# adelowo/cap

Hardware: AMD Instinct MI355X
Metric: verified JWTs/sec (RS256-2048, ES256) at 1/2/4/8 MI355X vs all-core Go CPU (higher is better)
Workload: dtype u32 (28-bit limbs, 64-bit v_mad_u64_u32 accumulators); 1 GPU; ES256 P-256 JWKS with 4 kids, 1M tokens batch-verified per MI355X (BASELINE configs[1]); kids=4, p256_key_comb_w=26, parallelism=independent shards x1

## Files before the change

### cap_amd/csrc/kernels/ec_small.hpp

```cpp
#pragma once
#include "ecdsa_impl.hpp"
#include "small_common.hpp"

namespace {

constexpr int SM_SPLIT = 16;
constexpr uint32_t SM_SIG_CHARS = 176;

__device__ __forceinline__ int sm_hash_bits(int alg) { return alg == 7 ? 256 : alg == 8 ? 384 : 512; }

template <class CV>
__device__ __forceinline__ void jadd_pair(JPt<typename CV::Fp>& P, int off, bool& exc) {
  using Fp = typename CV::Fp;
  constexpr int L = Fp::L;
  const bool lo = (threadIdx.x & off) == 0;
  uint32_t oz[L], ox[L], oy[L];
#pragma unroll
  for (int j = 0; j < L; ++j) {
    ox[j] = __shfl_xor(P.X[j], off);
    oy[j] = __shfl_xor(P.Y[j], off);
    oz[j] = __shfl_xor(P.Z[j], off);
  }
  const bool oinf = __shfl_xor((int)P.inf, off) != 0;
  const int pexc = __shfl_xor((int)exc, off);
// ... 126 lines not shown
  const bool size_ok = nch <= SM_SIG_CHARS && (nch & 3u) != 1u && D == 2u * (uint32_t)ks;
  if (wave == 1 && size_ok) {
    if (sm_b64_decode(sig_w, sig_shift, nch, sig_b, lane) && lane == 0) flag[0] = 1;
  }
  __syncthreads();

  if (wave == 1 && size_ok) {
    const int q = lane & 31, half = lane >> 5;
    if (q < CW) {
      uint32_t w = 0;
#pragma unroll
      for (int b = 0; b < 4; ++b) {
        const int pos = ks - 1 - (4 * q + b);
        if (pos >= 0) w |= (uint32_t)sig_b[half * ks + pos] << (8 * b);
      }
      if (4 * q + 4 > CB) {
        const uint32_t hi = 4 * q >= CB ? ~0u : ~0u << (8 * (CB - 4 * q));
        if (w & hi) flag[0] = 1;
      }
      rs_w[half * CW + q] = w;
    }
    for (int pos = lane; pos < ks - 4 * CW; pos += 64)
      if (sig_b[pos] != 0 || sig_b[ks + pos] != 0) flag[0] = 1;
  }
  SM_STAMP(2);
  __syncthreads();

  if (wave == 0 && lane == 0 && in_ok) {
    sm_hash(in_w, in_shift, jb.sig_in_len, sm_hash_bits(alg), dig_w);
  }
  uint32_t w[L];
  if (wave == 1 && lane < 4) {
    bool ok = size_ok && flag[0] == 0 && K.valid != 0 && (uint32_t)alg - 7u < 3u;
    uint32_t rw[CW], sw[CW], r[L], s[L], nl[L];
#pragma unroll
    for (int q = 0; q < CW; ++q) { rw[q] = rs_w[q]; sw[q] = rs_w[CW + q]; }
    mp::words_to_limbs<L, CW>(r, rw);
    mp::words_to_limbs<L, CW>(s, sw);
    mp::set_const<Fn>(nl, Fn::M);
    ok = ok && !zero_limbs<L>(r) && !zero_limbs<L>(s) && lt_limbs<L>(r, nl) && lt_limbs<L>(s, nl);
    if (ok) {
      uint32_t si[L], u2[L];
      mp::inv_plain_var4<Fn>(si, s);
      if (lane == 0) {
        mp::to_mont<Fn>(w, si);
        mp::mul<Fn>(u2, r, w); mp::csub<Fn>(u2);
#pragma unroll
        for (int j = 0; j < L; ++j) { sc[j] = r[j]; sc[2 * L + j] = u2[j]; }
        flag[1] = 1;
      }
    }
  }
  SM_STAMP(3);
  __syncthreads();
  const bool run = flag[1] != 0;

  if (run && wave == 1 && lane == 0) {
    constexpr int EW = ScalarRaw<CV>::EW;
    const int hw = ec_hash_words<CV>(alg);
    uint32_t ew[EW], e[L], u1[L], u2[L];
#pragma unroll
    for (int q = 0; q < EW; ++q) {
      const int src = hw - 1 - q;
      ew[q] = src >= 0 ? dig_w[src < 0 ? 0 : src] : 0u;
    }
    mp::words_to_limbs<L, EW>(e, ew);
    mp::csub<Fn>(e);
    mp::mul<Fn>(u1, e, w); mp::csub<Fn>(u1);
#pragma unroll
    for (int j = 0; j < L; ++j) { sc[L + j] = u1[j]; u2[j] = sc[2 * L + j]; }
    sm_recode<WG, NG, L>(u1, digs);
    sm_recode<WQ, NQ, L>(u2, digs + NG);
  }
  SM_STAMP(4);
  __syncthreads();

  SM_STAMP(5);
  if (wave != 0) return;
  JPt<Fp> P;
  P.inf = true;
#pragma unroll
  for (int j = 0; j < L; ++j) { P.X[j] = 0; P.Y[j] = 0; P.Z[j] = 0; }
  bool exc = false;
  const int sub = lane;
  if (run && sub < S) {
    const uint32_t* __restrict__ qtab = key_table(K);
    const uint32_t* __restrict__ gtab = a.gtab;
    uint32_t X[L], Y[L], Z[L];
    bool empty = true;
    constexpr int K = 2 * ((NWIN + S - 1) / S);
    constexpr int STRIDE = ec_stride(CV::CLS), NEG = ec_entries(CV::CLS, true), NEQ = 1 << (CV::WQ - 1);
    auto fetch = [&](int k, uint32_t* x, uint32_t* y) -> int {
      const int wi = sub + S * (k >> 1);
      const bool gen = (k & 1) == 0;
      if (wi >= (gen ? NG : NQ)) return 0;
      const int d = digs[gen ? wi : NG + wi];
      if (d == 0) return 0;
      const int ad = d < 0 ? -d : d;
      const uint32_t* ent = gen ? gtab + ((int64_t)wi * NEG + (ad - 1)) * STRIDE
                                : qtab + ((int64_t)wi * NEQ + (ad - 1)) * STRIDE;
      load_entry<CV>(ent, x, y);
      return d;
    };
    uint32_t xc[L], yc[L], xn[L], yn[L];
    int dc = fetch(0, xc, yc);
    int nadd = 0;
#pragma unroll
    for (int k = 0; k < K; ++k) {
      int dn = 0;
      if (k + 1 < K) dn = fetch(k + 1, xn, yn);
      if (dc != 0) {
        if (dc < 0) mp::neg<Fp>(yc, yc);
        if (empty) {
          mp::copy<Fp>(X, xc);
          mp::copy<Fp>(Y, yc); mp::freduce<Fp>(Y);
          mp::set_const<Fp>(Z, Fp::ONE);
          empty = false;
        } else if (nadd == 1) {
          madd_z1<Fp>(X, Y, Z, xc, yc);
        } else {
          madd<Fp>(X, Y, Z, xc, yc);
        }
        ++nadd;
      }
      if (k + 1 < K) {
        mp::copy<Fp>(xc, xn);
        mp::copy<Fp>(yc, yn);
        dc = dn;
      }
    }
    if (!empty) {
      mp::canon<Fp>(X); mp::canon<Fp>(Y); mp::canon<Fp>(Z);
      exc = mp::is_zero_canon<Fp>(Z);
      mp::copy<Fp>(P.X, X); mp::copy<Fp>(P.Y, Y); mp::copy<Fp>(P.Z, Z);
      P.inf = false;
    }
  }
  SM_STAMP(6);
#pragma unroll 1
  for (int off = 1; off < S; off <<= 1) jadd_pair<CV>(P, off, exc);
  if (lane != 0) return;
  SM_STAMP(7);
  bool ok = false;
  if (run) {
    uint32_t r[L];
#pragma unroll
    for (int j = 0; j < L; ++j) r[j] = sc[j];
    if (exc) {
      uint32_t u1[L], u2[L];
#pragma unroll
      for (int j = 0; j < L; ++j) { u1[j] = sc[L + j]; u2[j] = sc[2 * L + j]; }
      ok = ec_exact_ok<CV>(a.keyblob + K.aux_off, r, u1, u2);
    } else if (!P.inf) {
      ok = ec_x_matches<CV>(P.X, P.Z, r);
    }
  }
  a.verdict[a.out[blockIdx.x]] = ok ? 1 : 0;
#if JG_SMALL_PROF
  SM_STAMP(8);
  const uint64_t t0 = stamp[0][0];
  printf("smallprof w0 %lu %lu %lu %lu %lu %lu %lu %lu w1 %lu %lu %lu %lu %lu\n",
         stamp[0][1] - t0, stamp[0][2] - t0, stamp[0][3] - t0, stamp[0][4] - t0, stamp[0][5] - t0,
         stamp[0][6] - t0, stamp[0][7] - t0, stamp[0][8] - t0, stamp[1][1] - t0, stamp[1][2] - t0,
         stamp[1][3] - t0, stamp[1][4] - t0, stamp[1][5] - t0);
#endif
}

template <class CV>
void small_launch(const EcSmallArgs& a, hipStream_t s) {
  if (a.n == 0) return;
  hipLaunchKernelGGL(k_ec_small<CV>, dim3(a.n), dim3(SM_THREADS), 0, s, a);
}

}
```

### cap_amd/csrc/kernels/ecdsa.hpp

```cpp
#pragma once
#include <hip/hip_runtime.h>
#include <cstdint>

#include "common.hpp"
#include "point_form.hpp"
#include "prep.hpp"

struct EcArgs {
  const jgk::JobDev* jobs;
  const jgk::DevKey* keys;
  const uint32_t* keyblob;
  const uint32_t* sigw;
  const uint32_t* dig;
  uint8_t* status;
  uint8_t* verdict_pad;
  uint32_t* digs;
  uint32_t* u1w;
  uint32_t* u2w;
  const uint32_t* gtab;
  int32_t* exc_list;
  uint32_t* exc_count;
  int64_t npad, begin, end;
  int32_t wq;
  int32_t exc_reset;
  int32_t part;
  uint32_t* grp_next;
  int32_t point_blocks;
  int32_t force_point;
  int32_t point_exact;
};
enum : int32_t { EC_ALL = 0, EC_FAST = 1, EC_EXACT = 2 };

#ifndef JG_EC_POINT_SLOTS
#define JG_EC_POINT_SLOTS 4
#endif
static_assert(PF_CLS_P256 == jgk::CLS_P256 && PF_CLS_P384 == jgk::CLS_P384 && PF_CLS_P521 == jgk::CLS_P521 &&
              PF_CLS_ED25519 == jgk::CLS_ED25519, "point_form.hpp numbers the classes as common.hpp does");

constexpr int ec_limbs(int cls) { return cls == jgk::CLS_P256 ? 10 : cls == jgk::CLS_P384 ? 15 : 20; }
constexpr int ec_sig_words(int cls) { return cls == jgk::CLS_P256 ? 8 : cls == jgk::CLS_P384 ? 12 : 17; }
#ifndef JG_EC_PACK64
#define JG_EC_PACK64 1
#endif
constexpr bool ec_packed(int cls) { return JG_EC_PACK64 && cls == jgk::CLS_P256; }
constexpr int ec_stride(int cls) { return ec_packed(cls) ? 16 : (2 * ec_limbs(cls) + 3) & ~3; }
constexpr int ec_order_bits(int cls) { return cls == jgk::CLS_P256 ? 256 : cls == jgk::CLS_P384 ? 384 : 521; }
constexpr int ec_comb_w(int cls, bool gen) {
  return cls == jgk::CLS_P256 ? (gen ? 26 : 20) : cls == jgk::CLS_P384 ? (gen ? 24 : 16) : (gen ? 20 : 16);
}
constexpr int ec_windows_w(int cls, int w) { return (ec_order_bits(cls) + 2 + w - 1) / w; }
constexpr int ec_entries(int cls, bool gen) { return 1 << (ec_comb_w(cls, gen) - 1); }
constexpr int ec_windows(int cls, bool gen) { return ec_windows_w(cls, ec_comb_w(cls, gen)); }
constexpr int ec_digit_rows(int cls) { return ec_windows(cls, true) + ec_windows(cls, false); }
constexpr int ec_max_keys(int cls) { return 256; }
constexpr int64_t ec_table_words_w(int cls, int w) {
  return (int64_t)ec_windows_w(cls, w) * (1 << (w - 1)) * ec_stride(cls);
}
constexpr int64_t ec_table_words(int cls, bool gen) { return ec_table_words_w(cls, ec_comb_w(cls, gen)); }
constexpr int EC_P256_WQ[4] = {26, 24, 22, 20};
constexpr int EC_P384_WQ[4] = {24, 20, 18, 16};
constexpr int EC_P521_WQ[3] = {20, 18, 16};
constexpr bool ec_top_window_ok(int cls, int w) { return ec_order_bits(cls) - w * (ec_windows_w(cls, w) - 1) <= w - 2; }
static_assert(ec_top_window_ok(jgk::CLS_P256, 26) && ec_top_window_ok(jgk::CLS_P256, 24) &&
              ec_top_window_ok(jgk::CLS_P256, 22) && ec_top_window_ok(jgk::CLS_P256, 20) &&
              ec_top_window_ok(jgk::CLS_P384, 24) && ec_top_window_ok(jgk::CLS_P384, 20) &&
              ec_top_window_ok(jgk::CLS_P384, 18) && ec_top_window_ok(jgk::CLS_P384, 16) &&
              ec_top_window_ok(jgk::CLS_P521, 20) && ec_top_window_ok(jgk::CLS_P521, 18) &&
              ec_top_window_ok(jgk::CLS_P521, 16), "comb window count leaves no room for the top carry");

void launch_ec(int cls, const EcArgs& a, hipStream_t s, const jgk::Marker& mk);

constexpr int EC_SMALL_MAX = jgk::SMALL_MAX;
constexpr uint32_t EC_SMALL_IN_MAX = jgk::SMALL_IN_MAX;
struct EcSmallArgs {
  const uint8_t* arena;
  const jgk::DevKey* keys;
  const uint32_t* keyblob;
  const uint32_t* gtab;
  uint8_t* verdict;
  uint32_t n;
  jgk::JobDev jobs[EC_SMALL_MAX];
  uint16_t out[EC_SMALL_MAX];
};
void launch_ec_small(int cls, int wq, const EcSmallArgs& a, hipStream_t s);
void launch_ec_keyprep(int cls, jgk::DevKey* keys, uint32_t* blob, const int32_t* idx, int n, hipStream_t s);
void launch_ec_keytables(int cls, int wq, jgk::DevKey* keys, uint32_t* blob, const int32_t* tidx, int tn,
                         hipStream_t s, bool sliced = false);
void launch_ec_gtable(int cls, uint32_t* tab, hipStream_t s);
```

### cap_amd/csrc/kernels/ecdsa_impl.hpp

```cpp
#pragma once
#include <hip/hip_runtime.h>

#include <algorithm>
#include <cstdlib>
#include <type_traits>

#include "common.hpp"
#include "ecdsa.hpp"
#include "inv_shape.hpp"
#include "mp.hpp"
#include "tables.hpp"

using namespace jgk;

namespace {

template <int WQ_>
struct CurveP256W { using Fp = P256P; using Fn = P256N; using C = P256C; static constexpr int CLS = CLS_P256, WQ = WQ_; };
using CurveP256 = CurveP256W<20>;
template <int WQ_>
struct CurveP384W { using Fp = P384P; using Fn = P384N; using C = P384C; static constexpr int CLS = CLS_P384, WQ = WQ_; };
using CurveP384 = CurveP384W<16>;
template <int WQ_>
struct CurveP521W { using Fp = P521P; using Fn = P521N; using C = P521C; static constexpr int CLS = CLS_P521, WQ = WQ_; };
// ... 180 lines not shown
    const bool ok = ec_scalar_inputs<CV>(a, p, r, s, e);
    if (!ok && job_live(a.jobs[p])) a.status[p] = ST_REJECT;
    mp::to_mont<Fn>(sm, s);
    mp::mul<Fn>(acc, acc, sm);
#pragma unroll
    for (int k = 0; k < L; ++k) {
      a.u1w[(int64_t)k * np + p] = acc[k];
      a.u2w[(int64_t)k * np + p] = sm[k];
    }
    ++nb;
  }
  uint32_t inv[L];
  mp::block_inv<Fn, WPB>(inv, acc);
  for (int j = nb - 1; j >= 0; --j) {
    const int64_t p = a.begin + i + (int64_t)j * S;
    uint32_t cprev[L], sm[L], w[L];
    if (j > 0) {
      const int64_t pp = p - S;
#pragma unroll
      for (int k = 0; k < L; ++k) cprev[k] = a.u1w[(int64_t)k * np + pp];
    } else {
      mp::set_const<Fn>(cprev, Fn::ONE);
    }
#pragma unroll
    for (int k = 0; k < L; ++k) sm[k] = a.u2w[(int64_t)k * np + p];
    mp::mul<Fn>(w, inv, cprev);
    mp::mul<Fn>(inv, inv, sm);
    uint32_t r[L], e[L], u1[L], u2[L];
    ec_scalar_re<CV>(a, p, r, e);
    mp::mul<Fn>(u1, e, w); mp::csub<Fn>(u1);
    mp::mul<Fn>(u2, r, w); mp::csub<Fn>(u2);
    store_digit_rows<CV, WG, NG>(a, p, u1, 0);
    store_digit_rows<CV, WQ, NQ>(a, p, u2, NG);
  }
}

template <class Fp>
constexpr bool sum_ok() {
  if constexpr (std::is_same<Fp, P384P>::value) {
    return false;
  } else {
    uint32_t kmax = 0;
    for (int j = 0; j < Fp::L; ++j) kmax = Fp::KSUB[j] > kmax ? Fp::KSUB[j] : kmax;
    double red = 0;
    if constexpr (Fp::NP1)
      for (int j = 1; j < Fp::L; ++j) red += (double)Fp::M1[j] / 16777216.0;
    else
      red = 16.0 * Fp::L;
    return 9.0 * Fp::L + Fp::L * (double)kmax / 268435456.0 + red + 1.0 < 256.0;
  }
}

template <class Fp>
__device__ __forceinline__ void y3_from(uint32_t* Y, const uint32_t* r, const uint32_t* t, const uint32_t* y1,
                                        const uint32_t* hhh) {
  constexpr int L = Fp::L;
  if constexpr (sum_ok<Fp>() && mp::use_ps<Fp>(2)) {
    uint32_t ny1[L];
    mp::neg<Fp>(ny1, y1);
    mp::mont_ps<Fp, 2>(Y, r, t, ny1, hhh);
  } else if constexpr (sum_ok<Fp>()) {
    uint32_t ny1[L];
    mp::neg<Fp>(ny1, y1);
    uint64_t T[2 * L];
    mp::prod<Fp>(T, r, t);
    mp::prod_acc<Fp>(T, ny1, hhh);
    mp::mont_reduce<Fp>(Y, T);
  } else {
    uint32_t u[L];
    mp::mulf<Fp>(Y, r, t);
    mp::mulf<Fp>(u, y1, hhh);
    mp::sub<Fp>(Y, Y, u); mp::freduce_lazy<Fp>(Y);
  }
}

template <class Fp, class = void>
struct has_kx3 : std::false_type {};
template <class Fp>
struct has_kx3<Fp, std::void_t<decltype(Fp::KX3)>> : std::true_type {};

template <class Fp>
__device__ __forceinline__ void x3_from(uint32_t* X, const uint32_t* r, const uint32_t* hhh, const uint32_t* v) {
  constexpr int L = Fp::L;
  if constexpr (has_kx3<Fp>::value && mp::use_ps<Fp>(3)) {
    uint32_t e[L];
#pragma unroll
    for (int j = 0; j < L; ++j) e[j] = Fp::KX3[j] - (hhh[j] + 2 * v[j]);
    mp::mont_ps<Fp, 3>(X, r, r, nullptr, nullptr, e);
  } else if constexpr (has_kx3<Fp>::value) {
    uint64_t T[2 * L];
    mp::sqprod<Fp>(T, r);
    const uint32_t c1 = (uint32_t)mp::opaque_sgpr(1);
#pragma unroll
    for (int j = 0; j < L; ++j) T[L + j] += (uint64_t)(Fp::KX3[j] - (hhh[j] + 2 * v[j])) * c1;
    mp::mont_reduce<Fp>(X, T);
  } else {
    uint32_t r2[L];
    mp::sqrf<Fp>(r2, r);
    mp::sub<Fp>(X, r2, hhh); mp::sub<Fp>(X, X, v); mp::sub<Fp>(X, X, v); mp::freduce_lazy<Fp>(X);
  }
}

template <class Fp>
__device__ __forceinline__ void sub_x(uint32_t* r, const uint32_t* a, const uint32_t* x) {
  if constexpr (has_kx3<Fp>::value) {
#pragma unroll
    for (int j = 0; j < Fp::L; ++j) r[j] = a[j] + Fp::KSUBX[j] - x[j];
  } else {
    mp::sub<Fp>(r, a, x);
  }
}

template <class Fp>
__device__ __forceinline__ void madd(uint32_t* X, uint32_t* Y, uint32_t* Z, const uint32_t* x2, const uint32_t* y2) {
  constexpr int L = Fp::L;
  uint32_t z1z1[L], u2[L], t[L], s2[L], h[L], r[L], hh[L], hhh[L], v[L];
  mp::sqr_semi<Fp>(z1z1, Z);
  mp::mulf<Fp>(u2, x2, z1z1);
  mp::mulf<Fp>(t, Z, z1z1);
  mp::mulf<Fp>(s2, y2, t);
  sub_x<Fp>(h, u2, X);
  mp::sub<Fp>(r, s2, Y);
  mp::norm_for_mulf<Fp>(h);
  mp::norm_for_mulf<Fp>(r);
  mp::sqrf<Fp>(hh, h);
  mp::mulf<Fp>(Z, Z, h);
  mp::mulf<Fp>(hhh, h, hh);
  mp::mulf<Fp>(v, X, hh);
  uint32_t y1[L];
  mp::copy<Fp>(y1, Y);
  x3_from<Fp>(X, r, hhh, v);
  sub_x<Fp>(t, v, X);
  y3_from<Fp>(Y, r, t, y1, hhh);
}

template <class Fp>
__device__ __forceinline__ void madd_z1(uint32_t* X, uint32_t* Y, uint32_t* Z, const uint32_t* x2, const uint32_t* y2) {
  constexpr int L = Fp::L;
  uint32_t h[L], r[L], hh[L], hhh[L], v[L], t[L], y1[L];
  mp::sub<Fp>(h, x2, X);
  mp::sub<Fp>(r, y2, Y);
  mp::norm<Fp>(h);
  mp::norm<Fp>(r);
  mp::sqrf<Fp>(hh, h);
  mp::mulf<Fp>(hhh, h, hh);
  mp::mulf<Fp>(v, X, hh);
  mp::copy<Fp>(Z, h);
  mp::copy<Fp>(y1, Y);
  x3_from<Fp>(X, r, hhh, v);
  sub_x<Fp>(t, v, X);
  y3_from<Fp>(Y, r, t, y1, hhh);
}

template <class CV>
__device__ __forceinline__ void load_entry(const uint32_t* __restrict__ ent, uint32_t* x, uint32_t* y) {
  constexpr int L = CV::Fp::L;
  if constexpr (ec_packed(CV::CLS)) {
    const uint4* e4 = reinterpret_cast<const uint4*>(ent);
    const uint4 a = e4[0], b = e4[1], c = e4[2], d = e4[3];
    const uint32_t wx[8] = {a.x, a.y, a.z, a.w, b.x, b.y, b.z, b.w};
    const uint32_t wy[8] = {c.x, c.y, c.z, c.w, d.x, d.y, d.z, d.w};
    mp::words_to_limbs<L, 8>(x, wx);
    mp::words_to_limbs<L, 8>(y, wy);
  } else {
#pragma unroll
    for (int j = 0; j < L; ++j) { x[j] = ent[j]; y[j] = ent[L + j]; }
  }
}

template <class CV>
__device__ __forceinline__ void store_entry(uint32_t* out, const uint32_t* x, const uint32_t* y) {
  constexpr int L = CV::Fp::L;
  if constexpr (ec_packed(CV::CLS)) {
    uint32_t w[16];
    mp::limbs_to_words<L, 8>(w, x);
    mp::limbs_to_words<L, 8>(w + 8, y);
#pragma unroll
    for (int j = 0; j < 16; ++j) out[j] = w[j];
  } else {
#pragma unroll
    for (int j = 0; j < L; ++j) { out[j] = x[j]; out[L + j] = y[j]; }
  }
}

template <class CV>
struct RawEnt {
  static constexpr int NW = ec_packed(CV::CLS) ? 16 : 2 * CV::Fp::L;
  uint32_t w[NW];
};
template <class CV>
__device__ __forceinline__ void load_ent(RawEnt<CV>& r, const uint32_t* __restrict__ ent) {
  if constexpr (RawEnt<CV>::NW % 4 == 0) {
    const uint4* e4 = reinterpret_cast<const uint4*>(ent);
#pragma unroll
    for (int i = 0; i < RawEnt<CV>::NW / 4; ++i) {
      const uint4 q = e4[i];
      r.w[4 * i] = q.x; r.w[4 * i + 1] = q.y; r.w[4 * i + 2] = q.z; r.w[4 * i + 3] = q.w;
    }
  } else {
#pragma unroll
    for (int i = 0; i < RawEnt<CV>::NW; ++i) r.w[i] = ent[i];
  }
}
template <class CV, bool Z1ONE = false>
__device__ __forceinline__ void add_ent(uint32_t* X, uint32_t* Y, uint32_t* Z, bool& empty, const RawEnt<CV>& r, int d) {
  using Fp = typename CV::Fp;
  constexpr int L = Fp::L;
  if (d == 0) return;
  uint32_t x2[L], y2[L];
  if constexpr (ec_packed(CV::CLS)) {
    mp::words_to_limbs<L, 8>(x2, r.w);
    mp::words_to_limbs<L, 8>(y2, r.w + 8);
  } else {
#pragma unroll
    for (int j = 0; j < L; ++j) { x2[j] = r.w[j]; y2[j] = r.w[L + j]; }
  }
  if (d < 0) mp::neg<Fp>(y2, y2);
  if (empty) {
    mp::copy<Fp>(X, x2);
    mp::copy<Fp>(Y, y2); mp::freduce<Fp>(Y);
    mp::set_const<Fp>(Z, Fp::ONE);
    empty = false;
  } else if constexpr (Z1ONE) {
    madd_z1<Fp>(X, Y, Z, x2, y2);
  } else {
    madd<Fp>(X, Y, Z, x2, y2);
  }
}

template <class CV, bool GEN, bool Z1ONE = false>
__device__ __forceinline__ void add_window(uint32_t* X, uint32_t* Y, uint32_t* Z, bool& empty,
                                           const uint32_t* __restrict__ tab, int w, int d) {
  constexpr int STRIDE = ec_stride(CV::CLS), NE = GEN ? ec_entries(CV::CLS, true) : 1 << (CV::WQ - 1);
  if (d == 0) return;
  const int ad = d < 0 ? -d : d;
  RawEnt<CV> r;
  load_ent<CV>(r, tab + ((int64_t)w * NE + (ad - 1)) * STRIDE);
  add_ent<CV, Z1ONE>(X, Y, Z, empty, r, d);
}

template <class CV>
__device__ __forceinline__ void ec_load_r(const EcArgs& a, int64_t p, uint32_t* r) {
  constexpr int CW = ec_sig_words(CV::CLS);
  uint32_t rw[CW];
#pragma unroll
  for (int q = 0; q < CW; ++q) rw[q] = a.sigw[(int64_t)q * a.npad + p];
  mp::words_to_limbs<CV::Fp::L, CW>(r, rw);
}

template <class CV>
__device__ __forceinline__ bool ec_x_matches(const uint32_t* X, const uint32_t* Z, const uint32_t* r) {
  using Fp = typename CV::Fp;
  using Fn = typename CV::Fn;
  constexpr int L = Fp::L;
  uint32_t zz[L], rm[L], tt[L];
  mp::sqr<Fp>(zz, Z);
  mp::to_mont<Fp>(rm, r);
  mp::mul<Fp>(tt, rm, zz);
  bool ok = mp::eq_mod<Fp>(X, tt);
  if (!ok) {
    uint32_t rn[L], pl[L];
    mp::add<Fp>(rn, r, Fn::M);
    mp::norm<Fp>(rn);
    mp::set_const<Fp>(pl, Fp::M);
    if (lt_limbs<L>(rn, pl)) {
      mp::to_mont<Fp>(rm, rn);
      mp::mul<Fp>(tt, rm, zz);
      ok = mp::eq_mod<Fp>(X, tt);
    }
  }
  return ok;
}

template <class CV>
__device__ __forceinline__ void ec_point_token(const EcArgs& a, const int64_t p) {
  using Fp = typename CV::Fp;
  constexpr int L = Fp::L;
  constexpr int NG = ec_windows(CV::CLS, true), NQ = ec_windows_w(CV::CLS, CV::WQ);
  constexpr int NWIN = NG > NQ ? NG : NQ;
  const int64_t np = a.npad;
  const JobDev jb = a.jobs[p];
  if (!job_live(jb)) return;
  if (a.status[p] != ST_OK) { a.verdict_pad[p] = 0; return; }
  const int kidx = __builtin_amdgcn_readfirstlane(job_key(jb));
  const uint32_t* __restrict__ qtab = key_table(a.keys[kidx]);
  const uint32_t* __restrict__ gtab = a.gtab;

  uint32_t X[L], Y[L], Z[L];
  bool empty = true;
  add_window<CV, true>(X, Y, Z, empty, gtab, 0, (int)a.digs[p]);
  add_window<CV, false, true>(X, Y, Z, empty, qtab, 0, (int)a.digs[(int64_t)NG * np + p]);
  for (int w = 1; w < NWIN; ++w) {
    if (w < NG) add_window<CV, true>(X, Y, Z, empty, gtab, w, (int)a.digs[(int64_t)w * np + p]);
    if (w < NQ) add_window<CV, false>(X, Y, Z, empty, qtab, w, (int)a.digs[(int64_t)(NG + w) * np + p]);
  }
  if (empty) { a.verdict_pad[p] = 0; return; }
  uint32_t zc[L];
  mp::copy<Fp>(zc, Z);
  mp::canon<Fp>(zc);
  if (mp::is_zero_canon<Fp>(zc)) {
    const uint32_t idx = atomicAdd(a.exc_count, 1u);
    a.exc_list[idx] = (int32_t)p;
    a.status[p] = ST_EXCEPTIONAL;
    return;
  }
  uint32_t r[L];
  ec_load_r<CV>(a, p, r);
  a.verdict_pad[p] = ec_x_matches<CV>(X, Z, r);
}

template <class CV>
__global__ void __launch_bounds__(64) k_ec_point(EcArgs a) {
  if constexpr (!ec_point_persistent(CV::CLS)) {
    ec_point_token<CV>(a, a.begin + (int64_t)blockIdx.x * WAVE + threadIdx.x);
    return;
  }
  const uint32_t groups = (uint32_t)((a.end - a.begin) / WAVE);
  for (;;) {
    uint32_t g = 0;
    if (threadIdx.x == 0) g = atomicAdd(a.grp_next, 1u);
    g = __builtin_amdgcn_readfirstlane(g);
    if (g >= groups) return;
    ec_point_token<CV>(a, a.begin + (int64_t)g * WAVE + threadIdx.x);
  }
}

template <class Fp>
struct JPt { uint32_t X[Fp::L], Y[Fp::L], Z[Fp::L]; bool inf; };

template <class Fp>
__device__ bool is_zero_mod(const uint32_t* a) {
  uint32_t c[Fp::L];
  mp::copy<Fp>(c, a);
  mp::canon<Fp>(c);
  return mp::is_zero_canon<Fp>(c);
}

template <class Fp>
__device__ void times2(uint32_t* r, const uint32_t* a) {
  mp::add<Fp>(r, a, a);
  mp::freduce<Fp>(r);
}

template <class CV>
__device__ void jdbl(JPt<typename CV::Fp>& R, const JPt<typename CV::Fp>& P) {
  using Fp = typename CV::Fp;
  constexpr int L = Fp::L;
  if (P.inf || is_zero_mod<Fp>(P.Y)) { R.inf = true; return; }
  uint32_t delta[L], gamma[L], beta[L], t1[L], t2[L], alpha[L], b2[L], b4[L], b8[L], x3[L], y3[L], z3[L];
  mp::sqr<Fp>(delta, P.Z);
  mp::sqr<Fp>(gamma, P.Y);
  mp::mul<Fp>(beta, P.X, gamma);
  mp::sub<Fp>(t1, P.X, delta);
  mp::add<Fp>(t2, P.X, delta);
  mp::mul<Fp>(alpha, t1, t2);
  uint32_t three[L];
  mp::set_const<Fp>(three, CV::C::THREE_M);
  mp::mul<Fp>(alpha, alpha, three);
  times2<Fp>(b2, beta); times2<Fp>(b4, b2); times2<Fp>(b8, b4);
  mp::sqr<Fp>(x3, alpha);
  mp::sub<Fp>(x3, x3, b8); mp::freduce<Fp>(x3);
  mp::mul<Fp>(z3, P.Y, P.Z);
  times2<Fp>(z3, z3);
  mp::sub<Fp>(t1, b4, x3);
  mp::mul<Fp>(y3, alpha, t1);
  mp::sqr<Fp>(t2, gamma);
  times2<Fp>(t2, t2); times2<Fp>(t2, t2); times2<Fp>(t2, t2);
  mp::sub<Fp>(y3, y3, t2); mp::freduce<Fp>(y3);
  mp::copy<Fp>(R.X, x3); mp::copy<Fp>(R.Y, y3); mp::copy<Fp>(R.Z, z3);
  R.inf = false;
}

template <class CV>
__device__ void jadd(JPt<typename CV::Fp>& R, const JPt<typename CV::Fp>& P, const JPt<typename CV::Fp>& Q) {
  using Fp = typename CV::Fp;
  constexpr int L = Fp::L;
  if (P.inf) { R = Q; return; }
  if (Q.inf) { R = P; return; }
  uint32_t z1z1[L], z2z2[L], u1[L], u2[L], s1[L], s2[L], t[L], h[L], rr[L];
  mp::sqr<Fp>(z1z1, P.Z); mp::sqr<Fp>(z2z2, Q.Z);
  mp::mul<Fp>(u1, P.X, z2z2); mp::mul<Fp>(u2, Q.X, z1z1);
  mp::mul<Fp>(t, Q.Z, z2z2); mp::mul<Fp>(s1, P.Y, t);
  mp::mul<Fp>(t, P.Z, z1z1); mp::mul<Fp>(s2, Q.Y, t);
  mp::sub<Fp>(h, u2, u1); mp::freduce<Fp>(h);
  mp::sub<Fp>(rr, s2, s1); mp::freduce<Fp>(rr);
  if (is_zero_mod<Fp>(h)) {
    if (is_zero_mod<Fp>(rr)) { jdbl<CV>(R, P); return; }
    R.inf = true;
    return;
  }
  uint32_t hh[L], hhh[L], v[L], x3[L], y3[L], z3[L];
  mp::sqr<Fp>(hh, h); mp::mul<Fp>(hhh, h, hh); mp::mul<Fp>(v, u1, hh);
  mp::add<Fp>(t, hhh, v); mp::add<Fp>(t, t, v); mp::freduce<Fp>(t);
  mp::sqr<Fp>(x3, rr); mp::sub<Fp>(x3, x3, t); mp::freduce<Fp>(x3);
  mp::sub<Fp>(t, v, x3); mp::mul<Fp>(y3, rr, t);
  mp::mul<Fp>(t, s1, hhh); mp::sub<Fp>(y3, y3, t); mp::freduce<Fp>(y3);
  mp::mul<Fp>(t, P.Z, Q.Z); mp::mul<Fp>(z3, t, h);
  mp::copy<Fp>(R.X, x3); mp::copy<Fp>(R.Y, y3); mp::copy<Fp>(R.Z, z3);
  R.inf = false;
}

template <class CV>
__device__ void affine_point(JPt<typename CV::Fp>& P, const uint32_t* xm, const uint32_t* ym) {
  using Fp = typename CV::Fp;
  mp::copy<Fp>(P.X, xm); mp::copy<Fp>(P.Y, ym); mp::set_const<Fp>(P.Z, Fp::ONE);
  P.inf = false;
}

template <class CV>
__device__ bool ec_exact_ok(const uint32_t* aux, const uint32_t* r, const uint32_t* u1, const uint32_t* u2) {
  using Fp = typename CV::Fp;
  using Fn = typename CV::Fn;
  constexpr int L = Fp::L;
  {
    JPt<Fp> G, Q, GQ, R;
    uint32_t gx[L], gy[L];
    mp::set_const<Fp>(gx, CV::C::GX_M); mp::set_const<Fp>(gy, CV::C::GY_M);
    affine_point<CV>(G, gx, gy);
    affine_point<CV>(Q, aux, aux + L);
    jadd<CV>(GQ, G, Q);
    R.inf = true;
    for (int b = Fn::BITS - 1; b >= 0; --b) {
      jdbl<CV>(R, R);
      const int q = b / MP_W, sh = b % MP_W;
      const bool b1 = (u1[q] >> sh) & 1u, b2 = (u2[q] >> sh) & 1u;
      if (b1 && b2) jadd<CV>(R, R, GQ);
      else if (b1) jadd<CV>(R, R, G);
      else if (b2) jadd<CV>(R, R, Q);
    }
    bool ok = false;
    if (!R.inf) {
      uint32_t zi[L], zi2[L], xa[L], x[L];
      mp::inv<Fp>(zi, R.Z);
      mp::sqr<Fp>(zi2, zi);
      mp::mul<Fp>(xa, R.X, zi2);
      mp::from_mont<Fp>(x, xa);
      uint32_t nl[L], d[L];
      mp::set_const<Fp>(nl, Fn::M);
      if (!lt_limbs<L>(x, nl)) {
        int32_t br = 0;
#pragma unroll
        for (int j = 0; j < L; ++j) {
          const int32_t tt = (int32_t)x[j] - (int32_t)nl[j] + br;
          d[j] = (uint32_t)tt & MP_MASK;
          br = tt >> MP_W;
        }
        mp::copy<Fp>(x, d);
      }
      uint32_t o = 0;
#pragma unroll
      for (int j = 0; j < L; ++j) o |= x[j] ^ r[j];
      ok = o == 0;
    }
    return ok;
  }
}

template <class CV>
__global__ void __launch_bounds__(64) k_ec_exact(EcArgs a) {
  using Fn = typename CV::Fn;
  constexpr int L = Fn::L;
  const uint32_t cnt = *a.exc_count;
  for (uint32_t i = blockIdx.x * blockDim.x + threadIdx.x; i < cnt; i += gridDim.x * blockDim.x) {
    const int64_t p = a.exc_list[i];
    const int kidx = job_key(a.jobs[p]);
    const uint32_t* aux = a.keyblob + a.keys[kidx].aux_off;
    a.status[p] = ST_OK;
    uint32_t r[L], s[L], e[L], sm[L], w[L], u1[L], u2[L];
    (void)ec_scalar_inputs<CV>(a, p, r, s, e);
    mp::to_mont<Fn>(sm, s);
    mp::inv<Fn>(w, sm);
    mp::mul<Fn>(u1, e, w); mp::csub<Fn>(u1);
    mp::mul<Fn>(u2, r, w); mp::csub<Fn>(u2);
    a.verdict_pad[p] = ec_exact_ok<CV>(aux, r, u1, u2);
    a.status[p] = ST_OK;
  }
}

template <class CV, int S, bool PF>
__global__ void __launch_bounds__(64) k_ec_point_split(EcArgs a) {
  using Fp = typename CV::Fp;
  constexpr int L = Fp::L;
  constexpr int NG = ec_windows(CV::CLS, true), NQ = ec_windows_w(CV::CLS, CV::WQ);
  constexpr int NWIN = NG > NQ ? NG : NQ;
  const int lane = threadIdx.x, sub = lane % S;
  const int64_t p = a.begin + (int64_t)blockIdx.x * (WAVE / S) + lane / S;
  const int64_t np = a.npad;
  bool live = p < a.end;
  JobDev jb{};
  if (live) jb = a.jobs[p];
  live = live && job_live(jb);
  const bool ok_status = live && a.status[p] == ST_OK;
  if (live && !ok_status && sub == 0) a.verdict_pad[p] = 0;
  const bool run = ok_status;
  JPt<Fp> P;
  bool exc = false;
  P.inf = true;
  if (run) {
    const int kidx = job_key(jb);
    const uint32_t* __restrict__ qtab = key_table(a.keys[kidx]);
    const uint32_t* __restrict__ gtab = a.gtab;
    uint32_t X[L], Y[L], Z[L];
    bool empty = true;
    if constexpr (PF) {
      constexpr int STRIDE = ec_stride(CV::CLS), NEG = ec_entries(CV::CLS, true), NEQ = 1 << (CV::WQ - 1);
      const int nsteps = sub < NWIN ? 2 * ((NWIN - sub + S - 1) / S) : 0;
      auto dig = [&](int j) {
        const int w = sub + S * (j >> 1);
        const bool q = j & 1;
        return w < (q ? NQ : NG) ? (int)a.digs[(int64_t)(q ? NG + w : w) * np + p] : 0;
      };
      auto ent = [&](int j, int d) {
        const int ad = d < 0 ? -d : d;
        const int w = ad ? sub + S * (j >> 1) : 0;
        const int64_t i = ad ? ad - 1 : 0;
        return (j & 1) ? qtab + ((int64_t)w * NEQ + i) * STRIDE : gtab + ((int64_t)w * NEG + i) * STRIDE;
      };
      RawEnt<CV> rn;
      int dn = nsteps > 0 ? dig(0) : 0, dnn = nsteps > 1 ? dig(1) : 0;
      if (nsteps > 0) load_ent<CV>(rn, ent(0, dn));
#pragma unroll 1
      for (int j = 0; j < nsteps; ++j) {
        const RawEnt<CV> rc = rn;
        const int dc = dn;
        dn = dnn;
        if (j + 1 < nsteps) load_ent<CV>(rn, ent(j + 1, dn));
        if (j + 2 < nsteps) dnn = dig(j + 2);
        add_ent<CV>(X, Y, Z, empty, rc, dc);
      }
    } else {
      for (int w = sub; w < NWIN; w += S) {
        if (w < NG) add_window<CV, true>(X, Y, Z, empty, gtab, w, (int)a.digs[(int64_t)w * np + p]);
        if (w < NQ) add_window<CV, false>(X, Y, Z, empty, qtab, w, (int)a.digs[(int64_t)(NG + w) * np + p]);
      }
    }
    if (!empty) {
      mp::canon<Fp>(X); mp::canon<Fp>(Y); mp::canon<Fp>(Z);
      exc = mp::is_zero_canon<Fp>(Z);
      mp::copy<Fp>(P.X, X); mp::copy<Fp>(P.Y, Y); mp::copy<Fp>(P.Z, Z);
      P.inf = false;
    }
  }
#pragma unroll 1
  for (int off = 1; off < S; off <<= 1) {
    JPt<Fp> Q;
#pragma unroll
    for (int j = 0; j < L; ++j) {
      Q.X[j] = __shfl_xor(P.X[j], off);
      Q.Y[j] = __shfl_xor(P.Y[j], off);
      Q.Z[j] = __shfl_xor(P.Z[j], off);
    }
    Q.inf = __shfl_xor((int)P.inf, off) != 0;
    const int pexc = __shfl_xor((int)exc, off);
    exc = exc || pexc != 0;
    if (run && (sub & off) == 0 && !exc) jadd<CV>(P, P, Q);
  }
  if (!run || sub != 0) return;
  if (exc) {
    const uint32_t idx = atomicAdd(a.exc_count, 1u);
    a.exc_list[idx] = (int32_t)p;
    a.status[p] = ST_EXCEPTIONAL;
    return;
  }
  if (P.inf) { a.verdict_pad[p] = 0; return; }
  uint32_t r[L];
  ec_load_r<CV>(a, p, r);
  a.verdict_pad[p] = ec_x_matches<CV>(P.X, P.Z, r);
}

template <class CV>
__global__ void k_ec_keyprep(DevKey* keys, uint32_t* blob, const int32_t* idx, int n) {
  using Fp = typename CV::Fp;
  constexpr int L = Fp::L;
  const int i = blockIdx.x * blockDim.x + threadIdx.x;
  if (i >= n) return;
  DevKey& K = keys[idx[i]];
  uint32_t* aux = blob + K.aux_off;
  uint32_t x[L], y[L], pl[L];
#pragma unroll
  for (int j = 0; j < L; ++j) { x[j] = aux[j]; y[j] = aux[L + j]; }
  mp::set_const<Fp>(pl, Fp::M);
  bool ok = K.valid && lt_limbs<L>(x, pl) && lt_limbs<L>(y, pl);
  uint32_t xm[L], ym[L], lhs[L], rhs[L], t[L], three[L], b[L];
  mp::to_mont<Fp>(xm, x);
  mp::to_mont<Fp>(ym, y);
  mp::sqr<Fp>(lhs, ym);
  mp::sqr<Fp>(t, xm); mp::mul<Fp>(rhs, t, xm);
  mp::set_const<Fp>(three, CV::C::THREE_M);
  mp::mul<Fp>(t, xm, three);
  mp::sub<Fp>(rhs, rhs, t);
  mp::set_const<Fp>(b, CV::C::B_M);
  mp::add<Fp>(rhs, rhs, b);
  ok = ok && mp::eq_mod<Fp>(rhs, lhs);
  mp::canon<Fp>(xm); mp::canon<Fp>(ym);
#pragma unroll
  for (int j = 0; j < L; ++j) { aux[j] = xm[j]; aux[L + j] = ym[j]; }
  K.valid = ok ? 1 : 0;
}

template <class CV>
__device__ void store_affine(uint32_t* out, const JPt<typename CV::Fp>& P) {
  using Fp = typename CV::Fp;
  constexpr int L = Fp::L;
  uint32_t zi[L], zi2[L], zi3[L], x[L], y[L];
  mp::inv<Fp>(zi, P.Z);
  mp::sqr<Fp>(zi2, zi);
  mp::mul<Fp>(zi3, zi2, zi);
  mp::mul<Fp>(x, P.X, zi2);
  mp::mul<Fp>(y, P.Y, zi3);
  mp::canon<Fp>(x); mp::canon<Fp>(y);
  store_entry<CV>(out, x, y);
}

template <class CV, int W>
__device__ void window_base(uint32_t* out, const uint32_t* bx, const uint32_t* by, int w) {
  using Fp = typename CV::Fp;
  JPt<Fp> P;
  affine_point<CV>(P, bx, by);
  for (int i = 0; i < W * w; ++i) jdbl<CV>(P, P);
  store_affine<CV>(out, P);
}

template <class CV, int W>
__device__ void table_entry(uint32_t* out, const uint32_t* base, int d) {
  using Fp = typename CV::Fp;
  constexpr int L = Fp::L;
  JPt<Fp> P, acc;
  uint32_t bx[L], by[L];
  load_entry<CV>(base, bx, by);
  affine_point<CV>(P, bx, by);
  acc.inf = true;
  for (int bit = W - 1; bit >= 0; --bit) {
    jdbl<CV>(acc, acc);
    if ((d >> bit) & 1) jadd<CV>(acc, acc, P);
  }
  store_affine<CV>(out, acc);
}

template <class CV>
__global__ void k_ec_table_base_keys(const DevKey* keys, uint32_t* blob, const int32_t* idx, int n) {
  constexpr int W = CV::WQ, NWIN = ec_windows_w(CV::CLS, CV::WQ);
  constexpr int NE = 1 << (CV::WQ - 1), STRIDE = ec_stride(CV::CLS);
  const int w = blockIdx.x * blockDim.x + threadIdx.x;
  const int k = blockIdx.y;
  if (k >= n || w >= NWIN) return;
  const DevKey& K = keys[idx[k]];
  if (!K.valid) return;
  const uint32_t* aux = blob + K.aux_off;
  window_base<CV, W>((uint32_t*)K.tab + (int64_t)w * NE * STRIDE, aux, aux + CV::Fp::L, w);
}

template <class CV>
__global__ void k_ec_table_keys(const DevKey* keys, uint32_t* blob, const int32_t* idx, int n, int e0, int e1) {
  constexpr int W = CV::WQ, NWIN = ec_windows_w(CV::CLS, CV::WQ);
  constexpr int NE = 1 << (CV::WQ - 1), STRIDE = ec_stride(CV::CLS);
  const int e = e0 + blockIdx.x * blockDim.x + threadIdx.x;
  const int k = blockIdx.y;
  if (k >= n || e >= e1 || e >= NWIN * NE || e % NE == 0) return;
  const DevKey& K = keys[idx[k]];
  if (!K.valid) return;
  uint32_t* tab = (uint32_t*)K.tab;
  table_entry<CV, W>(tab + (int64_t)e * STRIDE, tab + (int64_t)(e / NE) * NE * STRIDE, e % NE + 1);
}

template <class CV>
__global__ void k_ec_table_base_g(uint32_t* tab) {
  constexpr int W = ec_comb_w(CV::CLS, true), NWIN = ec_windows(CV::CLS, true);
  constexpr int NE = ec_entries(CV::CLS, true), STRIDE = ec_stride(CV::CLS);
  using Fp = typename CV::Fp;
  const int w = blockIdx.x * blockDim.x + threadIdx.x;
  if (w >= NWIN) return;
  uint32_t gx[Fp::L], gy[Fp::L];
  mp::set_const<Fp>(gx, CV::C::GX_M); mp::set_const<Fp>(gy, CV::C::GY_M);
  window_base<CV, W>(tab + (int64_t)w * NE * STRIDE, gx, gy, w);
}

template <class CV>
__global__ void k_ec_table_g(uint32_t* tab) {
  constexpr int W = ec_comb_w(CV::CLS, true), NWIN = ec_windows(CV::CLS, true);
  constexpr int NE = ec_entries(CV::CLS, true), STRIDE = ec_stride(CV::CLS);
  const int e = blockIdx.x * blockDim.x + threadIdx.x;
  if (e >= NWIN * NE || e % NE == 0) return;
  table_entry<CV, W>(tab + (int64_t)e * STRIDE, tab + (int64_t)(e / NE) * NE * STRIDE, e % NE + 1);
}

template <class CV>
void launch_chain(const EcArgs& a, hipStream_t s, const Marker& mk) {
  const int64_t waves = (a.end - a.begin) / WAVE;
  dim3 g((unsigned)waves), b(WAVE);
  if (a.part == EC_EXACT) {
    hipLaunchKernelGGL(k_ec_exact<CV>, dim3(64), b, 0, s, a);
    mk("exact");
    return;
  }
  const int64_t n = a.end - a.begin;
  const InvShape sh = inv_shape(n, EC_SCALAR_WPB, EC_SCALAR_SOLO_MAX);
  if (sh.wpb == 1) {
    hipLaunchKernelGGL((k_ec_scalar_batch<CV, 1>), dim3(sh.grid), dim3(WAVE), 0, s, a, sh.B);
  } else {
    hipLaunchKernelGGL(k_ec_scalar_batch<CV>, dim3(sh.grid), dim3(WAVE * EC_SCALAR_WPB), 0, s, a, sh.B);
  }
  mk("scalar");
  const PointForm f = ec_point_form(CV::CLS, n, a.force_point != 0);
  const dim3 gs((unsigned)((n * f.lanes + WAVE - 1) / WAVE));
  if (f.lanes == EC_SPLIT && !f.prefetch) {
    hipLaunchKernelGGL((k_ec_point_split<CV, EC_SPLIT, false>), gs, b, 0, s, a);
  } else if (f.lanes == 2) {
    if constexpr (CV::CLS == jgk::CLS_P256) hipLaunchKernelGGL((k_ec_point_split<CV, 2, true>), gs, b, 0, s, a);
  } else if (f.prefetch) {
    hipLaunchKernelGGL((k_ec_point_split<CV, 1, true>), gs, b, 0, s, a);
  } else {
    if (f.persistent) {
      if (a.point_exact) g.x = (unsigned)a.point_blocks;
      else if (a.point_blocks > 0) g.x = (unsigned)std::min<int64_t>(waves, a.point_blocks);
    }
    hipLaunchKernelGGL(k_ec_point<CV>, g, b, 0, s, a);
  }
  mk("point");
  if (a.part == EC_FAST) return;
  hipLaunchKernelGGL(k_ec_exact<CV>, dim3(64), b, 0, s, a);
// ... 29 lines not shown
```

### cap_amd/csrc/kernels/ecdsa_p256.hip

```cpp
#include "ecdsa_impl.hpp"
#include "ec_small.hpp"

void launch_ec_p256(const EcArgs& a, hipStream_t s, const Marker& mk) {
  if (a.wq == 26) launch_chain<CurveP256W<26>>(a, s, mk);
  else if (a.wq == 24) launch_chain<CurveP256W<24>>(a, s, mk);
  else if (a.wq == 22) launch_chain<CurveP256W<22>>(a, s, mk);
  else launch_chain<CurveP256W<20>>(a, s, mk);
}

void launch_ec_keyprep_p256(DevKey* keys, uint32_t* blob, const int32_t* idx, int n, hipStream_t s) {
  keyprep_chain<CurveP256W<20>>(keys, blob, idx, n, s);
}

void launch_ec_keytables_p256(int wq, DevKey* keys, uint32_t* blob, const int32_t* tidx, int tn, hipStream_t s,
                              bool sliced) {
  if (wq == 26) keytables_chain<CurveP256W<26>>(keys, blob, tidx, tn, s, sliced);
  else if (wq == 24) keytables_chain<CurveP256W<24>>(keys, blob, tidx, tn, s, sliced);
  else if (wq == 22) keytables_chain<CurveP256W<22>>(keys, blob, tidx, tn, s, sliced);
  else keytables_chain<CurveP256W<20>>(keys, blob, tidx, tn, s, sliced);
}

void launch_ec_gtable_p256(uint32_t* tab, hipStream_t s) { gtable_chain<CurveP256W<20>>(tab, s); }

void launch_ec_small_p256(const EcSmallArgs& a, int wq, hipStream_t s) {
  if (wq == 26) small_launch<CurveP256W<26>>(a, s);
  else if (wq == 24) small_launch<CurveP256W<24>>(a, s);
  else if (wq == 22) small_launch<CurveP256W<22>>(a, s);
  else small_launch<CurveP256W<20>>(a, s);
}
```

### cap_amd/csrc/kernels/ecdsa_p384.hip

```cpp
#include "ecdsa_impl.hpp"
#include "ec_small.hpp"

void launch_ec_p384(const EcArgs& a, hipStream_t s, const Marker& mk) {
  if (a.wq == 24) launch_chain<CurveP384W<24>>(a, s, mk);
  else if (a.wq == 20) launch_chain<CurveP384W<20>>(a, s, mk);
  else if (a.wq == 18) launch_chain<CurveP384W<18>>(a, s, mk);
  else launch_chain<CurveP384W<16>>(a, s, mk);
}

void launch_ec_keyprep_p384(DevKey* keys, uint32_t* blob, const int32_t* idx, int n, hipStream_t s) {
  keyprep_chain<CurveP384W<16>>(keys, blob, idx, n, s);
}

void launch_ec_keytables_p384(int wq, DevKey* keys, uint32_t* blob, const int32_t* tidx, int tn, hipStream_t s,
                              bool sliced) {
  if (wq == 24) keytables_chain<CurveP384W<24>>(keys, blob, tidx, tn, s, sliced);
  else if (wq == 20) keytables_chain<CurveP384W<20>>(keys, blob, tidx, tn, s, sliced);
  else if (wq == 18) keytables_chain<CurveP384W<18>>(keys, blob, tidx, tn, s, sliced);
  else keytables_chain<CurveP384W<16>>(keys, blob, tidx, tn, s, sliced);
}

void launch_ec_gtable_p384(uint32_t* tab, hipStream_t s) { gtable_chain<CurveP384W<16>>(tab, s); }

void launch_ec_small_p384(const EcSmallArgs& a, int wq, hipStream_t s) {
  if (wq == 24) small_launch<CurveP384W<24>>(a, s);
  else if (wq == 20) small_launch<CurveP384W<20>>(a, s);
  else if (wq == 18) small_launch<CurveP384W<18>>(a, s);
  else small_launch<CurveP384W<16>>(a, s);
}
```

Before: 695.6 million verified JWTs/s.

## Use XYZZ coordinates for P-256 point accumulation and set waves-per-EU hint

```diff
diff --git a/cap_amd/csrc/kernels/ec_small.hpp b/cap_amd/csrc/kernels/ec_small.hpp
--- a/cap_amd/csrc/kernels/ec_small.hpp
+++ b/cap_amd/csrc/kernels/ec_small.hpp
@@ -302,7 +302,9 @@
       for (int j = 0; j < L; ++j) { u1[j] = sc[L + j]; u2[j] = sc[2 * L + j]; }
       ok = ec_exact_ok<CV>(a.keyblob + K.aux_off, r, u1, u2);
     } else if (!P.inf) {
-      ok = ec_x_matches<CV>(P.X, P.Z, r);
+      uint32_t zz[L];
+      mp::sqr<Fp>(zz, P.Z);
+      ok = ec_x_matches<CV>(P.X, zz, r);
     }
   }
   a.verdict[a.out[blockIdx.x]] = ok ? 1 : 0;
diff --git a/cap_amd/csrc/kernels/ecdsa.hpp b/cap_amd/csrc/kernels/ecdsa.hpp
--- a/cap_amd/csrc/kernels/ecdsa.hpp
+++ b/cap_amd/csrc/kernels/ecdsa.hpp
@@ -34,6 +34,7 @@
 #ifndef JG_EC_POINT_SLOTS
 #define JG_EC_POINT_SLOTS 4
 #endif
+constexpr bool ec_point_xyzz(int cls) { return cls == PF_CLS_P256; }
 static_assert(PF_CLS_P256 == jgk::CLS_P256 && PF_CLS_P384 == jgk::CLS_P384 && PF_CLS_P521 == jgk::CLS_P521 &&
               PF_CLS_ED25519 == jgk::CLS_ED25519, "point_form.hpp numbers the classes as common.hpp does");
 
diff --git a/cap_amd/csrc/kernels/ecdsa_impl.hpp b/cap_amd/csrc/kernels/ecdsa_impl.hpp
--- a/cap_amd/csrc/kernels/ecdsa_impl.hpp
+++ b/cap_amd/csrc/kernels/ecdsa_impl.hpp
@@ -356,6 +356,47 @@
   y3_from<Fp>(Y, r, t, y1, hhh);
 }
 
+template <class Fp>
+__device__ __forceinline__ void madd_xyzz(uint32_t* X, uint32_t* Y, uint32_t* ZZ, uint32_t* ZZZ, const uint32_t* x2,
+                                          const uint32_t* y2) {
+  constexpr int L = Fp::L;
+  uint32_t u2[L], s2[L], h[L], r[L], hh[L], hhh[L], v[L], t[L];
+  mp::mulf<Fp>(u2, x2, ZZ);
+  mp::mulf<Fp>(s2, y2, ZZZ);
+  sub_x<Fp>(h, u2, X);
+  mp::sub<Fp>(r, s2, Y);
+  mp::norm_for_mulf<Fp>(h);
+  mp::norm_for_mulf<Fp>(r);
+  mp::sqrf<Fp>(hh, h);
+  mp::mulf<Fp>(ZZ, ZZ, hh);
+  mp::mulf<Fp>(v, X, hh);
+  mp::mulf<Fp>(hhh, h, hh);
+  mp::mulf<Fp>(ZZZ, ZZZ, hhh);
+  uint32_t y1[L];
+  mp::copy<Fp>(y1, Y);
+  x3_from<Fp>(X, r, hhh, v);
+  sub_x<Fp>(t, v, X);
+  y3_from<Fp>(Y, r, t, y1, hhh);
+}
+
+template <class Fp>
+__device__ __forceinline__ void madd_xyzz_z1(uint32_t* X, uint32_t* Y, uint32_t* ZZ, uint32_t* ZZZ, const uint32_t* x2,
+                                             const uint32_t* y2) {
+  constexpr int L = Fp::L;
+  uint32_t h[L], r[L], v[L], t[L], y1[L];
+  mp::sub<Fp>(h, x2, X);
+  mp::sub<Fp>(r, y2, Y);
+  mp::norm<Fp>(h);
+  mp::norm<Fp>(r);
+  mp::sqrf<Fp>(ZZ, h);
+  mp::mulf<Fp>(ZZZ, h, ZZ);
+  mp::mulf<Fp>(v, X, ZZ);
+  mp::copy<Fp>(y1, Y);
+  x3_from<Fp>(X, r, ZZZ, v);
+  sub_x<Fp>(t, v, X);
+  y3_from<Fp>(Y, r, t, y1, ZZZ);
+}
+
 template <class CV>
 __device__ __forceinline__ void load_entry(const uint32_t* __restrict__ ent, uint32_t* x, uint32_t* y) {
   constexpr int L = CV::Fp::L;
@@ -406,8 +447,9 @@
     for (int i = 0; i < RawEnt<CV>::NW; ++i) r.w[i] = ent[i];
   }
 }
-template <class CV, bool Z1ONE = false>
-__device__ __forceinline__ void add_ent(uint32_t* X, uint32_t* Y, uint32_t* Z, bool& empty, const RawEnt<CV>& r, int d) {
+template <class CV, bool Z1ONE = false, bool XYZZ = false>
+__device__ __forceinline__ void add_ent(uint32_t* X, uint32_t* Y, uint32_t* Z, bool& empty, const RawEnt<CV>& r, int d,
+                                        uint32_t* ZZZ = nullptr) {
   using Fp = typename CV::Fp;
   constexpr int L = Fp::L;
   if (d == 0) return;
@@ -424,7 +466,11 @@
     mp::copy<Fp>(X, x2);
     mp::copy<Fp>(Y, y2); mp::freduce<Fp>(Y);
     mp::set_const<Fp>(Z, Fp::ONE);
+    if constexpr (XYZZ) mp::set_const<Fp>(ZZZ, Fp::ONE);
     empty = false;
+  } else if constexpr (XYZZ) {
+    if constexpr (Z1ONE) madd_xyzz_z1<Fp>(X, Y, Z, ZZZ, x2, y2);
+    else madd_xyzz<Fp>(X, Y, Z, ZZZ, x2, y2);
   } else if constexpr (Z1ONE) {
     madd_z1<Fp>(X, Y, Z, x2, y2);
   } else {
@@ -432,15 +478,15 @@
   }
 }
 
-template <class CV, bool GEN, bool Z1ONE = false>
+template <class CV, bool GEN, bool Z1ONE = false, bool XYZZ = false>
 __device__ __forceinline__ void add_window(uint32_t* X, uint32_t* Y, uint32_t* Z, bool& empty,
-                                           const uint32_t* __restrict__ tab, int w, int d) {
+                                           const uint32_t* __restrict__ tab, int w, int d, uint32_t* ZZZ = nullptr) {
   constexpr int STRIDE = ec_stride(CV::CLS), NE = GEN ? ec_entries(CV::CLS, true) : 1 << (CV::WQ - 1);
   if (d == 0) return;
   const int ad = d < 0 ? -d : d;
   RawEnt<CV> r;
   load_ent<CV>(r, tab + ((int64_t)w * NE + (ad - 1)) * STRIDE);
-  add_ent<CV, Z1ONE>(X, Y, Z, empty, r, d);
+  add_ent<CV, Z1ONE, XYZZ>(X, Y, Z, empty, r, d, ZZZ);
 }
 
 template <class CV>
@@ -453,12 +499,11 @@
 }
 
 template <class CV>
-__device__ __forceinline__ bool ec_x_matches(const uint32_t* X, const uint32_t* Z, const uint32_t* r) {
+__device__ __forceinline__ bool ec_x_matches(const uint32_t* X, const uint32_t* zz, const uint32_t* r) {
   using Fp = typename CV::Fp;
   using Fn = typename CV::Fn;
   constexpr int L = Fp::L;
-  uint32_t zz[L], rm[L], tt[L];
-  mp::sqr<Fp>(zz, Z);
+  uint32_t rm[L], tt[L];
   mp::to_mont<Fp>(rm, r);
   mp::mul<Fp>(tt, rm, zz);
   bool ok = mp::eq_mod<Fp>(X, tt);
@@ -490,13 +535,15 @@
   const uint32_t* __restrict__ qtab = key_table(a.keys[kidx]);
   const uint32_t* __restrict__ gtab = a.gtab;
 
-  uint32_t X[L], Y[L], Z[L];
+  constexpr bool XYZZ = ec_point_xyzz(CV::CLS);
+  uint32_t X[L], Y[L], Z[L], ZZZ[XYZZ ? L : 1];
   bool empty = true;
-  add_window<CV, true>(X, Y, Z, empty, gtab, 0, (int)a.digs[p]);
-  add_window<CV, false, true>(X, Y, Z, empty, qtab, 0, (int)a.digs[(int64_t)NG * np + p]);
+  add_window<CV, true, false, XYZZ>(X, Y, Z, empty, gtab, 0, (int)a.digs[p], ZZZ);
+  add_window<CV, false, true, XYZZ>(X, Y, Z, empty, qtab, 0, (int)a.digs[(int64_t)NG * np + p], ZZZ);
   for (int w = 1; w < NWIN; ++w) {
-    if (w < NG) add_window<CV, true>(X, Y, Z, empty, gtab, w, (int)a.digs[(int64_t)w * np + p]);
-    if (w < NQ) add_window<CV, false>(X, Y, Z, empty, qtab, w, (int)a.digs[(int64_t)(NG + w) * np + p]);
+    if (w < NG) add_window<CV, true, false, XYZZ>(X, Y, Z, empty, gtab, w, (int)a.digs[(int64_t)w * np + p], ZZZ);
+    if (w < NQ)
+      add_window<CV, false, false, XYZZ>(X, Y, Z, empty, qtab, w, (int)a.digs[(int64_t)(NG + w) * np + p], ZZZ);
   }
   if (empty) { a.verdict_pad[p] = 0; return; }
   uint32_t zc[L];
@@ -510,11 +557,20 @@
   }
   uint32_t r[L];
   ec_load_r<CV>(a, p, r);
-  a.verdict_pad[p] = ec_x_matches<CV>(X, Z, r);
-}
-
-template <class CV>
-__global__ void __launch_bounds__(64) k_ec_point(EcArgs a) {
+  if constexpr (XYZZ) {
+    a.verdict_pad[p] = ec_x_matches<CV>(X, Z, r);
+  } else {
+    uint32_t zz[L];
+    mp::sqr<Fp>(zz, Z);
+    a.verdict_pad[p] = ec_x_matches<CV>(X, zz, r);
+  }
+}
+
+#ifndef JG_EC_POINT_ATTR
+#define JG_EC_POINT_ATTR
+#endif
+template <class CV>
+__global__ void __launch_bounds__(64) JG_EC_POINT_ATTR k_ec_point(EcArgs a) {
   if constexpr (!ec_point_persistent(CV::CLS)) {
     ec_point_token<CV>(a, a.begin + (int64_t)blockIdx.x * WAVE + threadIdx.x);
     return;
@@ -769,7 +825,9 @@
   if (P.inf) { a.verdict_pad[p] = 0; return; }
   uint32_t r[L];
   ec_load_r<CV>(a, p, r);
-  a.verdict_pad[p] = ec_x_matches<CV>(P.X, P.Z, r);
+  uint32_t zz[L];
+  mp::sqr<Fp>(zz, P.Z);
+  a.verdict_pad[p] = ec_x_matches<CV>(P.X, zz, r);
 }
 
 template <class CV>
diff --git a/cap_amd/csrc/kernels/ecdsa_p256.hip b/cap_amd/csrc/kernels/ecdsa_p256.hip
--- a/cap_amd/csrc/kernels/ecdsa_p256.hip
+++ b/cap_amd/csrc/kernels/ecdsa_p256.hip
@@ -1,3 +1,4 @@
+#define JG_EC_POINT_ATTR __attribute__((amdgpu_waves_per_eu(4)))
 #include "ecdsa_impl.hpp"
 #include "ec_small.hpp"
 
diff --git a/cap_amd/csrc/kernels/ecdsa_p384.hip b/cap_amd/csrc/kernels/ecdsa_p384.hip
--- a/cap_amd/csrc/kernels/ecdsa_p384.hip
+++ b/cap_amd/csrc/kernels/ecdsa_p384.hip
@@ -1,3 +1,4 @@
+#define JG_EC_POINT_ATTR __attribute__((amdgpu_waves_per_eu(4)))
 #include "ecdsa_impl.hpp"
 #include "ec_small.hpp"
 
```

Measured after the change: 729.6 million verified JWTs/s, median of 6. +4.9%, better.
